# REXJJ/high-fidelity-pointcloud-fusion

Hardware: AMD Instinct MI355X
Metric: Mpts/s fused into 1 mm voxel grid (higher is better)
Workload: dtype f64

## Files before the change

### high-fidelity-pointcloud-fusion_amd/csrc/hfpf.hip

```cpp
#include <hip/hip_runtime.h>

#include <cstring>

#include <rocprim/rocprim.hpp>

#include <dlfcn.h>
#include <sched.h>
#include <sys/mman.h>

#if !defined(__HIP_DEVICE_COMPILE__)
#include <emmintrin.h>
#endif
#include <algorithm>
#include <atomic>
#include <condition_variable>
#include <cmath>
#include <cstdarg>
#include <cstdio>
#include <cstdlib>
#include <cstring>
#include <mutex>
#include <string>
#include <thread>
#include <vector>
// ... 151 lines not shown
{
    return DepthLayout{d.color_bpp ? (const uint8_t*)dev_color : nullptr, color_stride, d.width, d.depth_step, d.color_step, d.depth_f32,
                       d.color_bpp, d.color_bgr, d.cx, d.cy, d.sx, d.sy, d.unit};
}

struct Knobs {
    int copy_streams = 2;
    bool update_cells = true;
    int host_batch = 4;
    int upd_shape_forced = -1;
    bool trace_shape = false;
    bool bin_spare = true;
    bool stream_replay = true;
    float bin_slack = 2.0f;
    bool clean_small_nowait = true;
    float test_bin_scale = 1.f;
    bool test_table_skip = false;
    bool mailbox = true;
    int test_dev_tile = kDevTileDefault;
    int stage_threads = 0;
};

struct Session {
    bool dirty = false;
    uint64_t n_linked[kLogRegions] = {0};
    uint64_t gate_done = 0;
    bool pend_valid = false;
    uint64_t direct_linked = 0;
    bool normals_possible = false;
    uint32_t next_frame_id = 0;
    bool poisoned = false;
    std::string poison_msg;
    bool bin_have_hist = false;
    bool bin_from_probe = false;
    double bin_prev_points = 0;
    uint64_t n_bricks_known = 0;
    uint64_t n_bricks_before = 0;
    unsigned long long upd_miss_seen = 0, upd_member_seen = 0;
    unsigned long long pub_seq = 0;
    uint32_t pend_n = 0, pend_first = 0;
    uint32_t pend_pts = 0;
    uint32_t pend_lay[5] = {0, 0, 0, 0, 0};
    bool pend_depth = false;
    DepthSpec pend_ds{};
    double pend_pose[kFrameSlots * 12] = {0};
    uint64_t occ_exported = 0;
    uint64_t frames_exported = 0, frames_seen = 0;
};

constexpr int kTimeIntegrate = 0, kTimeClean = 1, kTimeDetail = 2, kTimeRaycast = 5, kTimeComponents = 6, kTimeCompare = 7, kTimedIds = 8;
struct TimedId {
    std::vector<std::pair<hipEvent_t, hipEvent_t>> pending;
    double ms = 0;
    uint64_t n = 0;
// ... 20 lines not shown
    uint32_t launch_seq = 0;
    bool upd_wide = false;
    bool epoch_used = false;
    unsigned long long mbox_seq = 0;
    int stage_next = 0, fslot_next = 0;

    Tables t;
    hipStream_t stream = nullptr;
    hipStream_t copy_stream = nullptr;
    hipStream_t copy_more[3] = {nullptr, nullptr, nullptr};
    std::vector<void*> allocs;
    uint64_t device_bytes = 0;
    unsigned long long* h_ctr = nullptr;
    unsigned long long* h_log_ctr = nullptr;
    unsigned long long* mbox = nullptr;
    std::vector<DevBuf*> bufs;
    DevBuf pend_a{bufs}, pend_b{bufs};
    StageSlot stage[kStageSlots];
    FrameSlot fslot[kFrameSlots];
    void* ring_d = nullptr;
    size_t ring_cap = 0;
    hipEvent_t busy_ev = nullptr;
    bool busy_pending = false;
    void* xfer_pin[2] = {nullptr, nullptr};
    hipEvent_t xfer_ev[2] = {nullptr, nullptr};
    StagePool* stage_pool = nullptr;
    DevBuf sort_tmp{bufs}, keys_a{bufs}, keys_b{bufs}, vals_a{bufs}, vals_b{bufs}, rows_dev{bufs};
    DevBuf probe_a{bufs}, probe_b{bufs}, probe_c{bufs}, probe_d{bufs}, probe_e{bufs}, probe_f{bufs};
    DevBuf result_out{bufs};
    DevBuf zbuf{bufs}, render_pose{bufs}, render_out{bufs};
// ... 104 lines not shown
    return HFPF_OK;
}

inline unsigned blocks_for(uint64_t n, unsigned bs) { return (unsigned)std::max<uint64_t>(1, (n + bs - 1) / bs); }

__global__ void k_set_ctr(unsigned long long* ctr, int idx, unsigned long long v) { ctr[idx] = v; }
__global__ void k_set_ctr3(unsigned long long* ctr, int i0, unsigned long long v0, int i1, unsigned long long v1, int i2, unsigned long long v2)
{
    ctr[i0] = v0;
    ctr[i1] = v1;
    if (i2 >= 0) ctr[i2] = v2;
}

constexpr int kMboxLogWords = 5;
constexpr int kMboxWords = C_COUNT + kLogRegions * kMboxLogWords;
__global__ __launch_bounds__(256) void k_publish_counters(const unsigned long long* __restrict__ ctr, const unsigned long long* __restrict__ log_ctr,
                                                          unsigned long long* mbox, unsigned long long seq)
{
    const unsigned i = threadIdx.x;
    if (i < (unsigned)C_COUNT) mbox[i] = ctr[i];
    for (unsigned w = i; w < (unsigned)(kLogRegions * kMboxLogWords); w += blockDim.x) mbox[C_COUNT + w] = log_ctr[(w / kMboxLogWords) * 16 + (w % kMboxLogWords)];
    __threadfence_system();
    __syncthreads();
    if (i == 0) __hip_atomic_store(&mbox[kMboxWords + 7], seq, __ATOMIC_RELEASE, __HIP_MEMORY_SCOPE_SYSTEM);
}

int read_counters(hfpf_handle* h)
{
    if (h->mbox) {
        unsigned long long seq = h->ss.pub_seq;
        h->ss.pub_seq = 0;
        if (seq == 0) {
            seq = ++h->mbox_seq;
            k_publish_counters<<<1, 256, 0, h->stream>>>(h->t.ctr, h->t.log_ctr, h->mbox, seq);
            HIPCHK(h, hipGetLastError());
        }
        volatile unsigned long long* flag = h->mbox + kMboxWords + 7;
        for (uint64_t spins = 1;; spins++) {
            if (__atomic_load_n(flag, __ATOMIC_ACQUIRE) == seq) break;
            __builtin_ia32_pause();
            if ((spins & 0xFFFF) == 0) {
                const hipError_t q = hipStreamQuery(h->stream);
                if (q != hipSuccess && q != hipErrorNotReady) HIPCHK(h, q);
                if (q == hipSuccess && __atomic_load_n(flag, __ATOMIC_ACQUIRE) != seq)
                    return fail(h, HFPF_ERR_HIP, "counter mailbox: the stream drained without publishing sequence %llu", seq);
            }
        }
        memcpy(h->h_ctr, h->mbox, C_COUNT * sizeof(unsigned long long));
        for (int r = 0; r < kLogRegions; r++)
            for (int w = 0; w < kMboxLogWords; w++) h->h_log_ctr[r * 16 + w] = h->mbox[C_COUNT + r * kMboxLogWords + w];
    } else {
        HIPCHK(h, hipMemcpyAsync(h->h_ctr, h->t.ctr, C_COUNT * sizeof(unsigned long long), hipMemcpyDeviceToHost, h->stream));
        HIPCHK(h, hipMemcpyAsync(h->h_log_ctr, h->t.log_ctr, kLogRegions * 16 * sizeof(unsigned long long), hipMemcpyDeviceToHost, h->stream));
        HIPCHK(h, hipStreamSynchronize(h->stream));
    }
    unsigned long long total = 0;
    for (int r = 0; r < kLogRegions; r++) total += std::min<unsigned long long>(h->h_log_ctr[r * 16], h->t.log_region_cap);
    h->h_ctr[C_LOG] = total;
    unsigned long long replayed = 0;
    for (int r = 0; r < kLogRegions; r++) replayed += h->h_log_ctr[r * 16 + 1];
    h->h_ctr[C_REPLAY_MEMBER] = replayed;
    unsigned long long upd_tested = 0, upd_member = 0;
    for (int r = 0; r < kLogRegions; r++) {
        upd_tested += h->h_log_ctr[r * 16 + 2];
        upd_member += h->h_log_ctr[r * 16 + 3];
// ... 33 lines not shown
float stat_scale_for(double bound) { return (float)std::ldexp(1.0, 26 - (int)std::floor(std::log2(bound))); }

Knobs read_knobs()
{
    Knobs k;
    if (const char* cs = getenv("HFPF_COPY_STREAMS")) k.copy_streams = std::max(1, std::min(atoi(cs), 4));
    const char* uf = getenv("HFPF_UPDATE_FORM");
    k.update_cells = !(uf && uf[0] == 'p');
    if (const char* hb = getenv("HFPF_HOST_BATCH")) k.host_batch = std::max(1, std::min(atoi(hb), kFrameSlots));
    if (const char* us = getenv("HFPF_UPD_SHAPE")) k.upd_shape_forced = std::max(0, std::min(atoi(us), 1));
    if (const char* tr = getenv("HFPF_TRACE_SHAPE")) k.trace_shape = tr[0] != '0';
    if (const char* sp = getenv("HFPF_BIN_SPARE")) k.bin_spare = sp[0] != '0';
    if (const char* sr = getenv("HFPF_STREAM_REPLAY")) k.stream_replay = sr[0] != '0';
    if (const char* bs = getenv("HFPF_BIN_SLACK")) k.bin_slack = std::max(1.0f, std::min(4.0f, (float)atof(bs)));
    if (const char* nw = getenv("HFPF_CLEAN_NOWAIT")) k.clean_small_nowait = nw[0] != '0';
    if (const char* bs = getenv("HFPF_TEST_BIN_SCALE")) k.test_bin_scale = std::max(0.f, std::min(1.f, (float)atof(bs)));
    const char* ts = getenv("HFPF_TEST_TABLE_SKIP");
    k.test_table_skip = ts && ts[0] == '1';
    if (const char* dt = getenv("HFPF_TEST_DEV_TILE")) k.test_dev_tile = std::max(8, std::min(atoi(dt), kDevTileMax));
    const char* mb = getenv("HFPF_MAILBOX");
    k.mailbox = !mb || mb[0] != '0';
    int cores = (int)std::thread::hardware_concurrency();
    cpu_set_t set;
    if (sched_getaffinity(0, sizeof set, &set) == 0) cores = std::min(cores > 0 ? cores : 1 << 20, CPU_COUNT(&set));
    const char* st = getenv("HFPF_STAGE_THREADS");
    k.stage_threads = st ? std::max(0, std::min(atoi(st), 15)) : std::max(0, std::min(7, cores / 2 - 1));
    return k;
}

int setup_params(hfpf_handle* h)
// ... 70 lines not shown
        memcpy(&g.d2_max, &lo_b, 4);
    }
    const double dir_entries = (double)g.bdim[0] * (double)g.bdim[1] * (double)g.bdim[2];
    if (dir_entries > 4.0e9) return fail(h, HFPF_ERR_BAD_CONFIG, "brick directory too large (%.3g entries)", dir_entries);
    h->dir_entries = (size_t)dir_entries;
    return HFPF_OK;
}

int reset_state(hfpf_handle* h, uint64_t bricks_used = ~0ull, uint64_t normals_used = ~0ull)
{
    Tables& t = h->t;
    hipStream_t s = h->stream;
    const uint64_t nb = std::min<uint64_t>(bricks_used, t.max_bricks);
    const uint64_t nsl = std::min<uint64_t>(h->n_slots, (nb + 1) * (uint64_t)kBrickCells);
    const uint64_t nn = std::min<uint64_t>(normals_used, t.max_normals);
    HIPCHK(h, hipMemsetAsync(t.dir, 0, h->dir_entries * 4, s));
    HIPCHK(h, hipMemsetAsync(t.info, 0, nsl * 8, s));
    HIPCHK(h, hipMemsetAsync(t.first_frame, 0xFF, nsl * 4, s));
    HIPCHK(h, hipMemsetAsync(t.buf_head, 0, nsl * 4 * kChains, s));
    HIPCHK(h, hipMemsetAsync(t.stat_id, 0, nsl * 4, s));
    HIPCHK(h, hipMemsetAsync(t.pre_dep, 0, nsl * 4, s));
    HIPCHK(h, hipMemsetAsync(t.dep_tmp, 0, nsl * 4, s));
    HIPCHK(h, hipMemsetAsync(t.occ_mask, 0, (nb + 1) * 8 * 8, s));
    HIPCHK(h, hipMemsetAsync(t.stats, 0, (nn + 1) * kStatWords * 8, s));
    HIPCHK(h, hipMemsetAsync(t.nd_mask, 0, (nb + 1) * 8 * 2 * 8, s));
    HIPCHK(h, hipMemsetAsync(t.ctr, 0, C_COUNT * 8, s));
    HIPCHK(h, hipMemsetAsync(t.log_ctr, 0, kLogRegions * 16 * 8, s));
    HIPCHK(h, hipMemsetAsync(t.bin_fill, 0, 2 * (t.max_bricks + 2) * 4, s));
    HIPCHK(h, hipMemsetAsync(t.bin_off, 0, 2 * (t.max_bricks + 2) * 4, s));
    HIPCHK(h, hipMemsetAsync(t.bin_capb, 0, 2 * (t.max_bricks + 2) * 4, s));
// ... 79 lines not shown
#define HFPF_SORT_BLOCK_ITEMS 4
#endif
using sort_config = rocprim::radix_sort_config<rocprim::default_config, rocprim::merge_sort_config<512, 1024, HFPF_SORT_BLOCK_ITEMS>, rocprim::default_config>;

template <typename Fn>
int with_sort_tmp(hfpf_handle* h, Fn&& fn)
{
    size_t bytes = 0;
    HIPCHK(h, fn((void*)nullptr, bytes));
    if (int rc = scratch(h, h->sort_tmp, bytes)) return rc;
    bytes = h->sort_tmp.bytes;
    HIPCHK(h, fn(h->sort_tmp.p, bytes));
    return HFPF_OK;
}

int sort_keys_u64(hfpf_handle* h, uint64_t* in, uint64_t* out, uint64_t n, unsigned bits = 0)
{
    const unsigned kb = bits ? bits : h->g.key_bits;
    return with_sort_tmp(h, [&](void* tmp, size_t& bytes) { return rocprim::radix_sort_keys<sort_config>(tmp, bytes, in, out, (size_t)n, 0, kb, h->stream); });
}

int sort_keys_u32(hfpf_handle* h, uint32_t* in, uint32_t* out, uint64_t n, unsigned bits = 32)
{
    return with_sort_tmp(h, [&](void* tmp, size_t& bytes) { return rocprim::radix_sort_keys<sort_config>(tmp, bytes, in, out, (size_t)n, 0, bits, h->stream); });
}

int sort_pairs_u64(hfpf_handle* h, uint64_t* kin, uint64_t* kout, uint32_t* vin, uint32_t* vout, uint64_t n, unsigned bits = 0)
{
    const unsigned kb = bits ? bits : h->g.key_bits;
    return with_sort_tmp(h, [&](void* tmp, size_t& bytes) {
        return rocprim::radix_sort_pairs<sort_config>(tmp, bytes, kin, kout, vin, vout, (size_t)n, 0, kb, h->stream);
    });
}

// ... 35 lines not shown
    if (s.cap < n_frames) {
        if (s.h_pose) {
            HIPCHK(h, hipHostFree(s.h_pose));
            HIPCHK(h, hipFree(s.d_pose));
            s.h_pose = nullptr, s.d_pose = nullptr, s.cap = 0;
        }
        const uint32_t cap = std::max<uint32_t>(n_frames, 64);
        const size_t bytes = (size_t)cap * (12 * sizeof(double) + sizeof(uint32_t));
        HIPCHK(h, hipHostMalloc((void**)&s.h_pose, bytes, hipHostMallocDefault));
        HIPCHK(h, hipMalloc((void**)&s.d_pose, bytes));
        s.cap = cap;
    }
    s.h_ids = reinterpret_cast<uint32_t*>(s.h_pose + 12 * (size_t)n_frames);
    s.d_ids = reinterpret_cast<uint32_t*>(s.d_pose + 12 * (size_t)n_frames);
    *out = &s;
    return HFPF_OK;
}

int pick_update_shape(hfpf_handle* h, double points, uint32_t nb)
{
    (void)points;
    (void)nb;
    if (h->knobs.upd_shape_forced >= 0) return h->knobs.upd_shape_forced;
    const unsigned long long miss = h->h_ctr[C_TABLE_MISS], member = h->h_ctr[C_DEP_MEMBER] + h->h_ctr[C_REPLAY_MEMBER];
    if (h->knobs.trace_shape)
        fprintf(stderr, "hfpf: update shape window: %llu table misses, %llu members (%llu of them replayed so far), %s\n", miss - std::min(miss, h->ss.upd_miss_seen),
                member - std::min(member, h->ss.upd_member_seen), h->h_ctr[C_REPLAY_MEMBER], h->upd_wide ? "wide" : "dense");
    if (!h->upd_wide && miss > h->ss.upd_miss_seen && (miss - h->ss.upd_miss_seen) * 500ull > member - std::min(member, h->ss.upd_member_seen)) h->upd_wide = true;
    h->ss.upd_miss_seen = miss;
    h->ss.upd_member_seen = member;
// ... 113 lines not shown
    return timed.file(id);
}

int integrate_device_locked(hfpf_handle* h, const void* dev_base, uint32_t n_frames, uint64_t frame_stride, uint32_t n_points,
                            uint32_t point_step, uint32_t off_x, uint32_t off_y, uint32_t off_z, uint32_t off_rgb, const double* poses,
                            const uint32_t* frame_ids, const DepthLayout* dl = nullptr)
{
    if (!dev_base || !poses || n_frames == 0) return fail(h, HFPF_ERR_BAD_ARG, "integrate: null buffer/poses or zero frames");
    if (n_points == 0) return HFPF_OK;
    const FrameLayout lay{point_step, off_x, off_y, off_z, off_rgb};
    if (!dl && (((uintptr_t)dev_base & 3) || (frame_stride & 3))) return fail(h, HFPF_ERR_BAD_ARG, "integrate: fields must be 4-byte aligned");
    int rc;
    if (!dl && (rc = check_cloud_layout(h, "integrate", lay, true))) return rc;
    if (n_frames > 65535) return fail(h, HFPF_ERR_BAD_ARG, "integrate: at most 65535 frames per call");
    h->ss.pub_seq = 0;
    StageSlot* s = nullptr;
    if ((rc = acquire_stage(h, n_frames, &s))) return rc;
    memcpy(s->h_pose, poses, (size_t)n_frames * 12 * sizeof(double));
    for (uint32_t f = 0; f < n_frames; f++) {
        const uint32_t id = frame_ids ? frame_ids[f] : h->ss.next_frame_id + f;
        if (id >= h->t.max_frames) return fail(h, HFPF_ERR_CAPACITY, "frame id %u >= max_frames %llu", id, (unsigned long long)h->t.max_frames);
        s->h_ids[f] = id;
    }
    if (!frame_ids) h->ss.next_frame_id += n_frames;
    HIPCHK(h, hipMemcpyAsync(s->d_pose, s->h_pose, (size_t)n_frames * (12 * sizeof(double) + sizeof(uint32_t)), hipMemcpyHostToDevice, h->stream));

    const int form = dl ? kFormDepth : packed16(lay, dev_base, true, frame_stride) ? kFormPacked16 : kFormStrided;
    const dim3 block(256);
    const uint64_t n_tiles = (uint64_t)blocks_for(n_points, 256) * n_frames;
    const uint32_t fw = dl ? dl->width : h->cfg.frame_width;
// ... 80 lines not shown
    const uint32_t log_rot = (uint32_t)((h->launch_seq++ * 17u) & (kLogRegions - 1));
    struct DetailGuard {
        hfpf_handle* h;
        size_t first;
        bool done = false;
        ~DetailGuard()
        {
            if (done) return;
            while (h->ev_detail.size() > first) {
                h->ev_free.push_back(h->ev_detail.back());
                h->ev_detail.pop_back();
            }
        }
    } detail_guard{h, h->ev_detail.size()};
    uint8_t detail_ran = 1;
    auto detail_mark = [&]() -> hipError_t {
        if (!h->timing_detail) return hipSuccess;
        hipEvent_t e = nullptr;
        if (hipError_t r = pooled_event(h, &e)) return r;
        h->ev_detail.push_back(e);
        return hipEventRecord(e, h->stream);
    };
    HIPCHK(h, detail_mark());
    launch_integrate(grid, bin, n_frames, log_rot, 0);
    if (!bin) {
        for (int k = 0; k < 3; k++) HIPCHK(h, detail_mark());
    } else {
        {
            const unsigned ogrid = (unsigned)std::min<uint64_t>(blocks_for((uint64_t)n_points * n_frames, 256), 8ull * 256);
            with_color(color, [&](auto C) { hipLaunchKernelGGL(k_integrate_overflow<C>, dim3(ogrid), dim3(256), 0, h->stream, h->g, h->t, log_rot); });
        }
        HIPCHK(h, detail_mark());
        if (have_plan) {
            if (h->h_ctr[C_NORMALS] > 0 || h->ss.normals_possible) {
                detail_ran |= 2;
                if (h->knobs.update_cells) {
                    const int shape = pick_update_shape(h, (double)n_points * n_frames, nb);
                    launch_update_cells<false>(color, shape == 1, h->stream, h->g, h->t, nb);
                } else {
                    with_color(color, [&](auto C) { hipLaunchKernelGGL(k_update<C>, dim3(nb), dim3(kUpdThreads), 0, h->stream, h->g, h->t, nb); });
                }
            }
            HIPCHK(h, detail_mark());
            detail_ran |= 4;
            with_color(color, [&](auto C) { hipLaunchKernelGGL(k_buffer<C>, dim3(nb), dim3(256), 0, h->stream, h->g, h->t, nb); });
            HIPCHK(h, detail_mark());
        } else {
            HIPCHK(h, detail_mark());
            HIPCHK(h, detail_mark());
        }
        h->ss.bin_have_hist = true;
        h->ss.bin_prev_points = (double)n_points * n_frames;
    }
    HIPCHK(h, hipGetLastError());
    if (h->timing_detail) h->ev_detail_ran.push_back(detail_ran);
    detail_guard.done = true;
    if ((rc = timed.file(kTimeIntegrate))) return rc;
    HIPCHK(h, hipEventRecord(s->done, h->stream));
    s->pending = true;
    h->ss.dirty = true;
    h->frames_integrated += n_frames;
    if (h->mbox && n_frames >= 4) {
        h->ss.pub_seq = ++h->mbox_seq;
        k_publish_counters<<<1, 256, 0, h->stream>>>(h->t.ctr, h->t.log_ctr, h->mbox, h->ss.pub_seq);
        HIPCHK(h, hipGetLastError());
    } else {
        h->ss.pub_seq = 0;
    }
    return HFPF_OK;
}

int resolve_timing(hfpf_handle* h)
{
    bool pending = !h->ev_detail.empty();
    for (const TimedId& t : h->timed) pending = pending || !t.pending.empty();
    if (!pending) return HFPF_OK;
    HIPCHK(h, hipStreamSynchronize(h->stream));
    for (TimedId& t : h->timed) {
        for (auto& pr : t.pending) {
            float ms = 0.f;
            HIPCHK(h, hipEventElapsedTime(&ms, pr.first, pr.second));
            t.ms += (double)ms;
            t.n++;
            h->ev_free.push_back(pr.first);
            h->ev_free.push_back(pr.second);
        }
        t.pending.clear();
    }
    for (size_t c = 0; 4 * c + 3 < h->ev_detail.size() && c < h->ev_detail_ran.size(); c++) {
        for (int k = 0; k < 3; k++) {
            if (!(h->ev_detail_ran[c] & (1u << k))) continue;
            float ms = 0.f;
            HIPCHK(h, hipEventElapsedTime(&ms, h->ev_detail[4 * c + k], h->ev_detail[4 * c + k + 1]));
            h->timed[kTimeDetail + k].ms += (double)ms;
            h->timed[kTimeDetail + k].n++;
        }
    }
    for (hipEvent_t e : h->ev_detail) h->ev_free.push_back(e);
    h->ev_detail.clear();
    h->ev_detail_ran.clear();
    return HFPF_OK;
}


typedef struct ncclComm* ncclComm_t_;
typedef struct { char internal[128]; } ncclUniqueId_;
enum { ncclSuccess_ = 0 };
enum { ncclChar_ = 0, ncclUint64_ = 5 };
// ... 149 lines not shown
    uint64_t maxc = 0;
    for (int r = 0; r < h->world; r++) maxc = std::max<uint64_t>(maxc, h->h_counts[r]);
    if (maxc == 0) return HFPF_OK;
    if (maxc > h->ex_cap_records) {
        const uint64_t new_cap = maxc + maxc / 4;
        const int grc = grow_exchange_buffers_locked(h, new_cap, n_mine);
        std::vector<unsigned long long> counts(h->h_counts, h->h_counts + h->world);
        if ((rc = dist_status_gather_locked(h, grc, new_cap, "growth of the exchange buffers", nullptr))) return rc;
        std::copy(counts.begin(), counts.end(), h->h_counts);
        h->ex_cap_records = new_cap;
    }
    NCCLCHK(h, g_rccl.AllGather(h->ex_send.p, h->ex_recv.p, maxc * sizeof(EpochRec), ncclChar_, (ncclComm_t_)h->comm, h->stream));
    return import_gathered_locked(h, h->ex_recv.p, maxc * sizeof(EpochRec), h->world, h->rank, h->h_counts);
}

void launch_gate(hfpf_handle* h, const uint32_t* cells_a, uint64_t n_a, const uint32_t* cells_b, uint64_t n_b, uint32_t* pend_out)
{
    const uint64_t n = n_a + n_b;
    if (n >= (1ull << 20))
        hipLaunchKernelGGL(k_gate<4>, dim3(blocks_for(n, 256 * 4)), dim3(256), 0, h->stream, h->g, h->t, cells_a, n_a, cells_b, n_b, pend_out);
    else
        hipLaunchKernelGGL(k_gate<1>, dim3(blocks_for(n, 256)), dim3(256), 0, h->stream, h->g, h->t, cells_a, n_a, cells_b, n_b, pend_out);
}

int clean_locked(hfpf_handle* h, int pre_rc)
{
    Tables& t = h->t;
    hipStream_t s = h->stream;
    int rc;
    if (h->dist_on && (rc = dist_exchange_locked(h, pre_rc))) return rc;
    if (pre_rc) return pre_rc;
    if ((rc = read_counters(h))) return rc;
    if ((rc = check_device_errors(h))) return rc;
    const uint64_t n_occ = std::min<uint64_t>(h->h_ctr[C_OCC], t.max_occ);
    const uint64_t n_normals = h->h_ctr[C_NORMALS];
    const uint64_t n_pend = h->ss.pend_valid ? h->h_ctr[C_PEND] : 0;
    h->ss.occ_exported = n_occ;
    h->ss.frames_exported = std::max(h->ss.frames_exported, h->ss.frames_seen);
    h->ss.dirty = false;
    h->clean_passes++;

    {
        LinkRanges lr;
        uint64_t max_new = 0;
        for (int r = 0; r < kLogRegions; r++) {
            const uint64_t n_r = std::min<uint64_t>(h->h_log_ctr[r * 16], t.log_region_cap);
            const uint64_t base = (uint64_t)r * t.log_region_cap;
// ... 6 lines not shown
            hipLaunchKernelGGL(k_link_log, dim3(blocks_for(max_new, 256), kLogRegions), dim3(256), 0, s, t, lr);
            HIPCHK(h, hipGetLastError());
        }
        h->ss.direct_linked = h->h_ctr[C_BUFFERED];
    }
    if (n_occ == 0) return HFPF_OK;

    const uint64_t n_new_occ = n_occ - std::min(n_occ, h->ss.gate_done);
    const uint64_t n_in = n_pend + n_new_occ;
    if (n_in == 0) return HFPF_OK;
    if ((rc = scratch(h, h->pend_b, n_in * 4))) return rc;
    if ((rc = scratch(h, h->keys_a, n_in * 8))) return rc;
    const uint64_t reg_ub = (2ull * (uint64_t)h->g.K + 1ull) * n_in;
    const uint64_t live_ub = std::min<uint64_t>(h->h_ctr[C_REG], t.max_reg) + std::min<uint64_t>(h->h_ctr[C_PREREG], t.max_reg);
    bool full = h->h_ctr[C_DEP] + 2 * live_ub + 2 * reg_ub + n_new_occ > t.max_dep;
    hipLaunchKernelGGL(k_clean_begin, dim3(blocks_for(n_in, 256)), dim3(256), 0, s, t, n_in, (const uint32_t*)(t.occ_list + h->ss.gate_done), n_new_occ, full ? 1u : 0u);
    launch_gate(h, (const uint32_t*)h->pend_a.p, n_pend, (const uint32_t*)(t.occ_list + h->ss.gate_done), n_new_occ, (uint32_t*)h->pend_b.p);
    HIPCHK(h, hipGetLastError());
    h->ss.gate_done = n_occ;
    h->ss.normals_possible = true;
    swap(h->pend_a, h->pend_b);
    h->ss.pend_valid = true;

    const unsigned cand_bits = HFPF_MORTON_IDS ? 3u * std::max(h->g.key_sy, std::max(h->g.key_sx - h->g.key_sy, h->g.key_bits - h->g.key_sx)) : h->g.key_bits;
    if ((rc = sort_keys_u64(h, t.cand_key, (uint64_t*)h->keys_a.p, n_in, cand_bits))) return rc;
    hipLaunchKernelGGL(k_normal, dim3(blocks_for(n_in, 128)), dim3(128), 0, s, h->g, t, (const uint64_t*)h->keys_a.p, kCountOnDevice, n_normals);
    const bool reg_small = n_in < (1ull << 18);
    const uint64_t reg_tile = 256ull * (reg_small ? kRegTilesSmall : kRegTilesLarge);
    const uint64_t reg_blocks = ((n_in + reg_tile - 1) / reg_tile) * (2ull * (uint64_t)h->g.K + 1ull);
    const uint32_t count_deps = full ? 0u : 1u;
    if (reg_small) hipLaunchKernelGGL(k_register<kRegTilesSmall>, dim3((unsigned)std::max<uint64_t>(reg_blocks, 1)), dim3(256), 0, s, h->g, t, kCountOnDevice, n_normals, count_deps);
    else hipLaunchKernelGGL(k_register<kRegTilesLarge>, dim3((unsigned)std::max<uint64_t>(reg_blocks, 1)), dim3(256), 0, s, h->g, t, kCountOnDevice, n_normals, count_deps);
    HIPCHK(h, hipGetLastError());
    uint64_t n_reg = 0, n_pre = 0, inc_touched = 0;
    const uint64_t reg_first = std::min<uint64_t>(h->h_ctr[C_REG], t.max_reg);
    const bool no_wait = !full && reg_ub < (1ull << 21) && h->knobs.clean_small_nowait;
    if (!full) {
        hipLaunchKernelGGL(k_depinc_offsets, dim3(blocks_for(reg_ub, 256 * kListTiles)), dim3(256), 0, s, t, kCountOnDevice);
        hipLaunchKernelGGL(k_depinc_fill, dim3(blocks_for(reg_ub, 256)), dim3(256), 0, s, t, reg_first, kCountOnDevice);
        HIPCHK(h, hipGetLastError());
        if (no_wait) {
            with_color(t.color, [&](auto C) {
                hipLaunchKernelGGL(k_replay<C>, dim3(blocks_for(reg_ub * kChains, 256)), dim3(256), 0, s, h->g, t, (const uint32_t*)t.touched_list, 1u, 0u,
                                   kCountOnDevice, n_normals);
            });
            HIPCHK(h, hipGetLastError());
            return HFPF_OK;
        }
// ... 96 lines not shown
    *out = nullptr;
    hfpf_handle* h = new hfpf_handle();
    h->cfg = *cfg;
    h->knobs = read_knobs();
    auto bail = [&](int rc) {
        g_create_error = h->err;
        for (void* p : h->allocs) (void)hipFree(p);
        for (DevBuf* b : h->bufs)
            if (b->p) (void)hipFree(b->p);
        if (h->h_ctr) (void)hipHostFree(h->h_ctr);
        if (h->h_log_ctr) (void)hipHostFree(h->h_log_ctr);
        if (h->mbox) (void)hipHostFree(h->mbox);
        if (h->copy_stream) (void)hipStreamDestroy(h->copy_stream);
        for (hipStream_t cs : h->copy_more)
            if (cs) (void)hipStreamDestroy(cs);
        if (h->stream) (void)hipStreamDestroy(h->stream);
        delete h;
        return rc;
    };
    int rc = setup_params(h);
    if (rc) return bail(rc);
    int ndev = 0;
    hipError_t e = hipGetDeviceCount(&ndev);
    if (e != hipSuccess || ndev <= 0) return bail(fail(h, HFPF_ERR_HIP, "no HIP device available (%s); this engine has no CPU path", hipGetErrorString(e)));
    if (cfg->device < 0 || cfg->device >= ndev) return bail(fail(h, HFPF_ERR_BAD_CONFIG, "device %d out of range (%d devices)", cfg->device, ndev));
    if ((e = hipSetDevice(cfg->device)) != hipSuccess) return bail(fail(h, HFPF_ERR_HIP, "hipSetDevice: %s", hipGetErrorString(e)));
    if ((e = hipStreamCreateWithFlags(&h->stream, hipStreamNonBlocking)) != hipSuccess) return bail(fail(h, HFPF_ERR_HIP, "hipStreamCreate: %s", hipGetErrorString(e)));
    if ((e = hipStreamCreateWithFlags(&h->copy_stream, hipStreamNonBlocking)) != hipSuccess) return bail(fail(h, HFPF_ERR_HIP, "hipStreamCreate: %s", hipGetErrorString(e)));
    for (int k = 0; k + 1 < h->knobs.copy_streams; k++)
        if ((e = hipStreamCreateWithFlags(&h->copy_more[k], hipStreamNonBlocking)) != hipSuccess) return bail(fail(h, HFPF_ERR_HIP, "hipStreamCreate: %s", hipGetErrorString(e)));
    if ((e = hipHostMalloc((void**)&h->h_ctr, C_COUNT * sizeof(unsigned long long), hipHostMallocDefault)) != hipSuccess)
        return bail(fail(h, HFPF_ERR_HIP, "hipHostMalloc: %s", hipGetErrorString(e)));
    memset(h->h_ctr, 0, C_COUNT * sizeof(unsigned long long));
    if ((e = hipHostMalloc((void**)&h->h_log_ctr, kLogRegions * 16 * sizeof(unsigned long long), hipHostMallocDefault)) != hipSuccess)
        return bail(fail(h, HFPF_ERR_HIP, "hipHostMalloc: %s", hipGetErrorString(e)));
    memset(h->h_log_ctr, 0, kLogRegions * 16 * sizeof(unsigned long long));
    if (h->knobs.mailbox) {
        if ((e = hipHostMalloc((void**)&h->mbox, (kMboxWords + 8) * sizeof(unsigned long long), hipHostMallocCoherent | hipHostMallocMapped)) != hipSuccess)
            return bail(fail(h, HFPF_ERR_HIP, "hipHostMalloc (mailbox): %s", hipGetErrorString(e)));
        memset(h->mbox, 0, (kMboxWords + 8) * sizeof(unsigned long long));
    }
    {
        int per_cu = 0, cus = 0;
        hipDeviceProp_t prop;
        if (hipGetDeviceProperties(&prop, cfg->device) == hipSuccess) cus = prop.multiProcessorCount;
        if (hipOccupancyMaxActiveBlocksPerMultiprocessor(&per_cu, h->binned ? k_integrate<true, false, true> : k_integrate<true, false, false>, 256, 0) != hipSuccess) per_cu = 4;
        h->integrate_grid = std::max(1, per_cu) * std::max(1, cus);
    }
    if ((rc = alloc_tables(h))) return bail(rc);
    {
        const uint64_t n0 = h->cfg.max_normals;
        if ((rc = scratch(h, h->keys_a, n0 * 8)) || (rc = scratch(h, h->keys_b, n0 * 8)) || (rc = scratch(h, h->vals_a, n0 * 4)) ||
            (rc = scratch(h, h->vals_b, n0 * 4)) || (rc = scratch(h, h->pend_b, n0 * 4)) || (rc = scratch(h, h->sort_tmp, n0 * 16)))
            return bail(rc);
        if (h->cfg.max_call_points && h->binned) {
// ... 11 lines not shown
            if (h->xfer_pin[0]) (void)hipHostFree(h->xfer_pin[0]);
            h->xfer_pin[0] = nullptr;
            break;
        }
    }
    if ((e = hipStreamSynchronize(h->stream)) != hipSuccess) return bail(fail(h, HFPF_ERR_HIP, "sync after init: %s", hipGetErrorString(e)));
    *out = h;
    return HFPF_OK;
}

int hfpf_destroy(hfpf_handle* h)
{
    if (!h) return HFPF_OK;
    (void)hipSetDevice(h->cfg.device);
    (void)hipStreamSynchronize(h->stream);
    for (void* p : h->allocs) (void)hipFree(p);
    for (DevBuf* b : h->bufs)
        if (b->p) (void)hipFree(b->p);
    if (h->comm && g_rccl.CommDestroy) (void)g_rccl.CommDestroy((ncclComm_t_)h->comm);
    if (h->h_counts) (void)hipHostFree(h->h_counts);
    for (auto& s : h->stage) {
        if (s.h_pose) (void)hipHostFree(s.h_pose);
        if (s.d_pose) (void)hipFree(s.d_pose);
        if (s.done) (void)hipEventDestroy(s.done);
    }
    delete h->stage_pool;
    h->stage_pool = nullptr;
    for (int k = 0; k < 2; k++) {
        if (h->xfer_pin[k]) (void)hipHostFree(h->xfer_pin[k]);
        if (h->xfer_ev[k]) (void)hipEventDestroy(h->xfer_ev[k]);
// ... 12 lines not shown
    for (hipStream_t cs : h->copy_more)
        if (cs) {
            (void)hipStreamSynchronize(cs);
            (void)hipStreamDestroy(cs);
        }
    for (TimedId& t : h->timed)
        for (auto& pr : t.pending) {
            (void)hipEventDestroy(pr.first);
            (void)hipEventDestroy(pr.second);
        }
    for (auto e : h->ev_detail) (void)hipEventDestroy(e);
    for (auto e : h->ev_free) (void)hipEventDestroy(e);
    if (h->h_ctr) (void)hipHostFree(h->h_ctr);
    if (h->h_log_ctr) (void)hipHostFree(h->h_log_ctr);
    if (h->mbox) (void)hipHostFree(h->mbox);
    if (h->stream) (void)hipStreamDestroy(h->stream);
    delete h;
    return HFPF_OK;
}

int hfpf_get_dims(const hfpf_handle* h, int32_t dims[3], double* resolution)
{
    if (!h) return HFPF_ERR_BAD_ARG;
    if (dims) memcpy(dims, h->g.dim, 3 * sizeof(int32_t));
    if (resolution) *resolution = h->g.res;
    return HFPF_OK;
}

static int flush_pending_locked(hfpf_handle* h);

// ... 3176 lines not shown
```

### high-fidelity-pointcloud-fusion_amd/csrc/kernels.hpp

```cpp
#pragma once
#include <type_traits>

#include "stats.hpp"

namespace hfpf {

typedef float vf4 __attribute__((ext_vector_type(4)));

struct FrameLayout {
    uint32_t point_step, off_x, off_y, off_z, off_rgb;
};

struct DepthLayout {
    const uint8_t* color;
    uint64_t color_stride;
    uint32_t width, depth_step, color_step;
    uint32_t depth_f32;
    uint32_t color_bpp;
    uint32_t color_bgr;
    float cx, cy, sx, sy, unit;
};

template <bool WANT_RGB>
__device__ __forceinline__ vf4 depth_fetch(const uint8_t* __restrict__ dimg, const uint8_t* __restrict__ cimg, const DepthLayout& L, uint32_t i)
// ... 1236 lines not shown
    block_reserve_tiles<TILES>(&t.ctr[C_CAND], n_pass, ci, trs);
    block_reserve_tiles<TILES>(&t.ctr[C_PEND], n_pend, pi, trs);
#pragma unroll
    for (int tt = 0; tt < TILES; tt++) {
        if (n_pass[tt]) t.cand_key[ci[tt]] = key_[tt];
        if (n_pend[tt]) pend_out[pi[tt]] = slot_[tt];
    }
}

__device__ __forceinline__ uint64_t cand_count(const Tables& t, uint64_t base)
{
    const uint64_t n = t.ctr[C_CAND];
    const uint64_t room = t.max_normals > base ? t.max_normals - base : 0;
    return n < room ? n : room;
}
__global__ __launch_bounds__(256) void k_clean_begin(const Tables t, const uint64_t n_in, const uint32_t* __restrict__ new_cells, const uint64_t n_new,
                                                     const uint32_t lists_only)
{
    const uint64_t i = (uint64_t)blockIdx.x * blockDim.x + threadIdx.x;
    if (i < n_in) t.cand_key[i] = ~0ull;
    if (i == 0) {
        t.ctr[C_CAND] = 0;
        t.ctr[C_PEND] = 0;
        t.ctr[C_TOUCHED] = 0;
    }
    if (i < (uint64_t)kLogRegions) t.log_ctr[i * 16 + 4] = 0;
    if ((uint64_t)blockIdx.x * blockDim.x >= n_new) return;
    uint32_t slot = 0, nid = 0;
    if (i < n_new) {
        slot = new_cells[i];
        nid = t.pre_dep[slot];
    }
    __shared__ BlockReserveScratch brs;
    const unsigned long long li = block_reserve(&t.ctr[C_PREREG], nid != 0, brs);
    const unsigned long long off = lists_only ? 0ull : block_reserve(&t.ctr[C_DEP], nid != 0, brs);
    if (!nid) return;
    if (li < t.max_reg) t.prereg_list[li] = slot;
    else atomicOr(&t.ctr[C_ERR], (unsigned long long)E_REG);
    set_dep_flag(t, slot);
    if (lists_only) return;
    if (off >= t.max_dep) {
        atomicOr(&t.ctr[C_ERR], (unsigned long long)E_DEP);
        return;
    }
    t.dep[off] = make_dep_entry(t, nid);
    t.info[slot] = (t.info[slot] & 3ull) | (1ull << kDepCntShift) | ((uint64_t)off << kDepOffShift);
}

__global__ __launch_bounds__(128) void k_normal(const GridParams g, const Tables t, const uint64_t* __restrict__ sorted_keys,
                                                const uint64_t n_cand_arg, const uint64_t base)
{
    const uint64_t n_cand = n_cand_arg == kCountOnDevice ? cand_count(t, base) : n_cand_arg;
    const uint64_t r = (uint64_t)blockIdx.x * blockDim.x + threadIdx.x;
    if (r == 0 && n_cand_arg == kCountOnDevice) {
        if (t.ctr[C_CAND] > n_cand) atomicOr(&t.ctr[C_ERR], (unsigned long long)E_NORMALS);
        t.ctr[C_NORMALS] = base + n_cand;
    }
    if (r >= n_cand) return;
    int32_t x, y, z;
    uint64_t key = sorted_keys[r];
    if (HFPF_MORTON_IDS) {
// ... 2584 lines not shown
```

Baseline: 28120.

## Overlap clean front half with update-cells kernel on a second stream

Result: faster. 29420 (median of 6 runs) (+4.6%).

```diff
diff --git a/high-fidelity-pointcloud-fusion_amd/csrc/hfpf.hip b/high-fidelity-pointcloud-fusion_amd/csrc/hfpf.hip
--- a/high-fidelity-pointcloud-fusion_amd/csrc/hfpf.hip
+++ b/high-fidelity-pointcloud-fusion_amd/csrc/hfpf.hip
@@ -189,6 +189,8 @@
     bool stream_replay = true;
     float bin_slack = 2.0f;
     bool clean_small_nowait = true;
+    bool clean_overlap = true;
+    bool trace_clean = false;
     float test_bin_scale = 1.f;
     bool test_table_skip = false;
     bool mailbox = true;
@@ -213,6 +215,8 @@
     uint64_t n_bricks_before = 0;
     unsigned long long upd_miss_seen = 0, upd_member_seen = 0;
     unsigned long long pub_seq = 0;
+    unsigned long long early_seq = 0;
+    unsigned long long win_seq = 0;
     uint32_t pend_n = 0, pend_first = 0;
     uint32_t pend_pts = 0;
     uint32_t pend_lay[5] = {0, 0, 0, 0, 0};
@@ -263,6 +267,8 @@
     unsigned long long* h_ctr = nullptr;
     unsigned long long* h_log_ctr = nullptr;
     unsigned long long* mbox = nullptr;
+    hipStream_t front_stream = nullptr;
+    hipEvent_t ev_ready = nullptr, ev_front = nullptr;
     std::vector<DevBuf*> bufs;
     DevBuf pend_a{bufs}, pend_b{bufs};
     StageSlot stage[kStageSlots];
@@ -397,6 +403,7 @@
 
 constexpr int kMboxLogWords = 5;
 constexpr int kMboxWords = C_COUNT + kLogRegions * kMboxLogWords;
+constexpr int kMboxSlotWords = (kMboxWords + 8 + 7) & ~7;
 __global__ __launch_bounds__(256) void k_publish_counters(const unsigned long long* __restrict__ ctr, const unsigned long long* __restrict__ log_ctr,
                                                           unsigned long long* mbox, unsigned long long seq)
 {
@@ -408,30 +415,39 @@
     if (i == 0) __hip_atomic_store(&mbox[kMboxWords + 7], seq, __ATOMIC_RELEASE, __HIP_MEMORY_SCOPE_SYSTEM);
 }
 
-int read_counters(hfpf_handle* h)
+int await_mailbox(hfpf_handle* h, const unsigned long long* box, unsigned long long seq)
+{
+    const unsigned long long* flag = box + kMboxWords + 7;
+    for (uint64_t spins = 1;; spins++) {
+        if (__atomic_load_n(flag, __ATOMIC_ACQUIRE) == seq) break;
+        __builtin_ia32_pause();
+        if ((spins & 0xFFFF) == 0) {
+            const hipError_t q = hipStreamQuery(h->stream);
+            if (q != hipSuccess && q != hipErrorNotReady) HIPCHK(h, q);
+            if (q == hipSuccess && __atomic_load_n(flag, __ATOMIC_ACQUIRE) != seq)
+                return fail(h, HFPF_ERR_HIP, "counter mailbox: the stream drained without publishing sequence %llu", seq);
+        }
+    }
+    return HFPF_OK;
+}
+
+int read_counters(hfpf_handle* h, bool early = false)
 {
     if (h->mbox) {
-        unsigned long long seq = h->ss.pub_seq;
+        unsigned long long seq = early ? h->ss.early_seq : h->ss.pub_seq;
+        const unsigned long long* box = h->mbox + (early ? kMboxSlotWords : 0);
+        h->ss.win_seq = early ? h->ss.pub_seq : 0;
         h->ss.pub_seq = 0;
+        h->ss.early_seq = 0;
         if (seq == 0) {
             seq = ++h->mbox_seq;
             k_publish_counters<<<1, 256, 0, h->stream>>>(h->t.ctr, h->t.log_ctr, h->mbox, seq);
             HIPCHK(h, hipGetLastError());
         }
-        volatile unsigned long long* flag = h->mbox + kMboxWords + 7;
-        for (uint64_t spins = 1;; spins++) {
-            if (__atomic_load_n(flag, __ATOMIC_ACQUIRE) == seq) break;
-            __builtin_ia32_pause();
-            if ((spins & 0xFFFF) == 0) {
-                const hipError_t q = hipStreamQuery(h->stream);
-                if (q != hipSuccess && q != hipErrorNotReady) HIPCHK(h, q);
-                if (q == hipSuccess && __atomic_load_n(flag, __ATOMIC_ACQUIRE) != seq)
-                    return fail(h, HFPF_ERR_HIP, "counter mailbox: the stream drained without publishing sequence %llu", seq);
-            }
-        }
-        memcpy(h->h_ctr, h->mbox, C_COUNT * sizeof(unsigned long long));
+        if (int rc = await_mailbox(h, box, seq)) return rc;
+        memcpy(h->h_ctr, box, C_COUNT * sizeof(unsigned long long));
         for (int r = 0; r < kLogRegions; r++)
-            for (int w = 0; w < kMboxLogWords; w++) h->h_log_ctr[r * 16 + w] = h->mbox[C_COUNT + r * kMboxLogWords + w];
+            for (int w = 0; w < kMboxLogWords; w++) h->h_log_ctr[r * 16 + w] = box[C_COUNT + r * kMboxLogWords + w];
     } else {
         HIPCHK(h, hipMemcpyAsync(h->h_ctr, h->t.ctr, C_COUNT * sizeof(unsigned long long), hipMemcpyDeviceToHost, h->stream));
         HIPCHK(h, hipMemcpyAsync(h->h_log_ctr, h->t.log_ctr, kLogRegions * 16 * sizeof(unsigned long long), hipMemcpyDeviceToHost, h->stream));
@@ -495,6 +511,8 @@
     if (const char* sr = getenv("HFPF_STREAM_REPLAY")) k.stream_replay = sr[0] != '0';
     if (const char* bs = getenv("HFPF_BIN_SLACK")) k.bin_slack = std::max(1.0f, std::min(4.0f, (float)atof(bs)));
     if (const char* nw = getenv("HFPF_CLEAN_NOWAIT")) k.clean_small_nowait = nw[0] != '0';
+    if (const char* co = getenv("HFPF_CLEAN_OVERLAP")) k.clean_overlap = co[0] != '0';
+    if (const char* tc = getenv("HFPF_TRACE_CLEAN")) k.trace_clean = tc[0] != '0';
     if (const char* bs = getenv("HFPF_TEST_BIN_SCALE")) k.test_bin_scale = std::max(0.f, std::min(1.f, (float)atof(bs)));
     const char* ts = getenv("HFPF_TEST_TABLE_SKIP");
     k.test_table_skip = ts && ts[0] == '1';
@@ -595,6 +613,7 @@
     const uint64_t nb = std::min<uint64_t>(bricks_used, t.max_bricks);
     const uint64_t nsl = std::min<uint64_t>(h->n_slots, (nb + 1) * (uint64_t)kBrickCells);
     const uint64_t nn = std::min<uint64_t>(normals_used, t.max_normals);
+    if (h->front_stream) HIPCHK(h, hipStreamSynchronize(h->front_stream));
     HIPCHK(h, hipMemsetAsync(t.dir, 0, h->dir_entries * 4, s));
     HIPCHK(h, hipMemsetAsync(t.info, 0, nsl * 8, s));
     HIPCHK(h, hipMemsetAsync(t.first_frame, 0xFF, nsl * 4, s));
@@ -704,10 +723,11 @@
     return HFPF_OK;
 }
 
-int sort_keys_u64(hfpf_handle* h, uint64_t* in, uint64_t* out, uint64_t n, unsigned bits = 0)
+int sort_keys_u64(hfpf_handle* h, uint64_t* in, uint64_t* out, uint64_t n, unsigned bits = 0, hipStream_t on = nullptr)
 {
     const unsigned kb = bits ? bits : h->g.key_bits;
-    return with_sort_tmp(h, [&](void* tmp, size_t& bytes) { return rocprim::radix_sort_keys<sort_config>(tmp, bytes, in, out, (size_t)n, 0, kb, h->stream); });
+    const hipStream_t st = on ? on : h->stream;
+    return with_sort_tmp(h, [&](void* tmp, size_t& bytes) { return rocprim::radix_sort_keys<sort_config>(tmp, bytes, in, out, (size_t)n, 0, kb, st); });
 }
 
 int sort_keys_u32(hfpf_handle* h, uint32_t* in, uint32_t* out, uint64_t n, unsigned bits = 32)
@@ -773,6 +793,24 @@
     s.h_ids = reinterpret_cast<uint32_t*>(s.h_pose + 12 * (size_t)n_frames);
     s.d_ids = reinterpret_cast<uint32_t*>(s.d_pose + 12 * (size_t)n_frames);
     *out = &s;
+    return HFPF_OK;
+}
+
+int window_from_final(hfpf_handle* h)
+{
+    const unsigned long long seq = h->ss.win_seq;
+    h->ss.win_seq = 0;
+    if (!seq || !h->mbox) return HFPF_OK;
+    if (int rc = await_mailbox(h, h->mbox, seq)) return rc;
+    unsigned long long member = h->mbox[C_DEP_MEMBER], tested = h->mbox[C_DEP_TESTED];
+    for (int r = 0; r < kLogRegions; r++) {
+        tested += h->mbox[C_COUNT + r * kMboxLogWords + 2];
+        member += h->mbox[C_COUNT + r * kMboxLogWords + 3];
+    }
+    h->h_ctr[C_DEP_TESTED] = tested;
+    h->h_ctr[C_DEP_MEMBER] = member;
+    h->h_ctr[C_TABLE_MISS] = h->mbox[C_TABLE_MISS];
+    h->h_ctr[C_UPD_ROUNDS] = h->mbox[C_UPD_ROUNDS];
     return HFPF_OK;
 }
 
@@ -916,6 +954,7 @@
     if (!dl && (rc = check_cloud_layout(h, "integrate", lay, true))) return rc;
     if (n_frames > 65535) return fail(h, HFPF_ERR_BAD_ARG, "integrate: at most 65535 frames per call");
     h->ss.pub_seq = 0;
+    h->ss.early_seq = 0;
     StageSlot* s = nullptr;
     if ((rc = acquire_stage(h, n_frames, &s))) return rc;
     memcpy(s->h_pose, poses, (size_t)n_frames * 12 * sizeof(double));
@@ -1026,6 +1065,7 @@
         }
     } detail_guard{h, h->ev_detail.size()};
     uint8_t detail_ran = 1;
+    unsigned long long early_seq = 0;
     auto detail_mark = [&]() -> hipError_t {
         if (!h->timing_detail) return hipSuccess;
         hipEvent_t e = nullptr;
@@ -1044,9 +1084,25 @@
         }
         HIPCHK(h, detail_mark());
         if (have_plan) {
-            if (h->h_ctr[C_NORMALS] > 0 || h->ss.normals_possible) {
+            const bool update = h->h_ctr[C_NORMALS] > 0 || h->ss.normals_possible;
+            const bool buffer_first = update && h->knobs.clean_overlap && h->mbox && n_frames >= 4 && !h->dist_on;
+            auto launch_buffer = [&]() {
+                detail_ran |= 4;
+                with_color(color, [&](auto C) { hipLaunchKernelGGL(k_buffer<C>, dim3(nb), dim3(256), 0, h->stream, h->g, h->t, nb); });
+            };
+            if (buffer_first) {
+                detail_ran |= 8;
+                launch_buffer();
+                early_seq = ++h->mbox_seq;
+                k_publish_counters<<<1, 256, 0, h->stream>>>(h->t.ctr, h->t.log_ctr, h->mbox + kMboxSlotWords, early_seq);
+                HIPCHK(h, hipGetLastError());
+                HIPCHK(h, hipEventRecord(h->ev_ready, h->stream));
+                HIPCHK(h, detail_mark());
+            }
+            if (update) {
                 detail_ran |= 2;
                 if (h->knobs.update_cells) {
+                    if ((rc = window_from_final(h))) return rc;
                     const int shape = pick_update_shape(h, (double)n_points * n_frames, nb);
                     launch_update_cells<false>(color, shape == 1, h->stream, h->g, h->t, nb);
                 } else {
@@ -1054,9 +1110,10 @@
                 }
             }
             HIPCHK(h, detail_mark());
-            detail_ran |= 4;
-            with_color(color, [&](auto C) { hipLaunchKernelGGL(k_buffer<C>, dim3(nb), dim3(256), 0, h->stream, h->g, h->t, nb); });
-            HIPCHK(h, detail_mark());
+            if (!buffer_first) {
+                launch_buffer();
+                HIPCHK(h, detail_mark());
+            }
         } else {
             HIPCHK(h, detail_mark());
             HIPCHK(h, detail_mark());
@@ -1073,9 +1130,11 @@
     h->ss.dirty = true;
     h->frames_integrated += n_frames;
     if (h->mbox && n_frames >= 4) {
+        if ((rc = window_from_final(h))) return rc;
         h->ss.pub_seq = ++h->mbox_seq;
         k_publish_counters<<<1, 256, 0, h->stream>>>(h->t.ctr, h->t.log_ctr, h->mbox, h->ss.pub_seq);
         HIPCHK(h, hipGetLastError());
+        h->ss.early_seq = early_seq;
     } else {
         h->ss.pub_seq = 0;
     }
@@ -1102,8 +1161,9 @@
     for (size_t c = 0; 4 * c + 3 < h->ev_detail.size() && c < h->ev_detail_ran.size(); c++) {
         for (int k = 0; k < 3; k++) {
             if (!(h->ev_detail_ran[c] & (1u << k))) continue;
+            const int at = (k && (h->ev_detail_ran[c] & 8u)) ? 3 - k : k;
             float ms = 0.f;
-            HIPCHK(h, hipEventElapsedTime(&ms, h->ev_detail[4 * c + k], h->ev_detail[4 * c + k + 1]));
+            HIPCHK(h, hipEventElapsedTime(&ms, h->ev_detail[4 * c + at], h->ev_detail[4 * c + at + 1]));
             h->timed[kTimeDetail + k].ms += (double)ms;
             h->timed[kTimeDetail + k].n++;
         }
@@ -1283,13 +1343,13 @@
     return import_gathered_locked(h, h->ex_recv.p, maxc * sizeof(EpochRec), h->world, h->rank, h->h_counts);
 }
 
-void launch_gate(hfpf_handle* h, const uint32_t* cells_a, uint64_t n_a, const uint32_t* cells_b, uint64_t n_b, uint32_t* pend_out)
+void launch_gate(hfpf_handle* h, hipStream_t s, const uint32_t* cells_a, uint64_t n_a, const uint32_t* cells_b, uint64_t n_b, uint32_t* pend_out)
 {
     const uint64_t n = n_a + n_b;
     if (n >= (1ull << 20))
-        hipLaunchKernelGGL(k_gate<4>, dim3(blocks_for(n, 256 * 4)), dim3(256), 0, h->stream, h->g, h->t, cells_a, n_a, cells_b, n_b, pend_out);
+        hipLaunchKernelGGL(k_gate<4>, dim3(blocks_for(n, 256 * 4)), dim3(256), 0, s, h->g, h->t, cells_a, n_a, cells_b, n_b, pend_out);
     else
-        hipLaunchKernelGGL(k_gate<1>, dim3(blocks_for(n, 256)), dim3(256), 0, h->stream, h->g, h->t, cells_a, n_a, cells_b, n_b, pend_out);
+        hipLaunchKernelGGL(k_gate<1>, dim3(blocks_for(n, 256)), dim3(256), 0, s, h->g, h->t, cells_a, n_a, cells_b, n_b, pend_out);
 }
 
 int clean_locked(hfpf_handle* h, int pre_rc)
@@ -1299,7 +1359,8 @@
     int rc;
     if (h->dist_on && (rc = dist_exchange_locked(h, pre_rc))) return rc;
     if (pre_rc) return pre_rc;
-    if ((rc = read_counters(h))) return rc;
+    const bool early = h->knobs.clean_overlap && !h->dist_on && h->binned && h->mbox && h->ss.pub_seq && h->ss.early_seq;
+    if ((rc = read_counters(h, early))) return rc;
     if ((rc = check_device_errors(h))) return rc;
     const uint64_t n_occ = std::min<uint64_t>(h->h_ctr[C_OCC], t.max_occ);
     const uint64_t n_normals = h->h_ctr[C_NORMALS];
@@ -1336,8 +1397,19 @@
     const uint64_t reg_ub = (2ull * (uint64_t)h->g.K + 1ull) * n_in;
     const uint64_t live_ub = std::min<uint64_t>(h->h_ctr[C_REG], t.max_reg) + std::min<uint64_t>(h->h_ctr[C_PREREG], t.max_reg);
     bool full = h->h_ctr[C_DEP] + 2 * live_ub + 2 * reg_ub + n_new_occ > t.max_dep;
-    hipLaunchKernelGGL(k_clean_begin, dim3(blocks_for(n_in, 256)), dim3(256), 0, s, t, n_in, (const uint32_t*)(t.occ_list + h->ss.gate_done), n_new_occ, full ? 1u : 0u);
-    launch_gate(h, (const uint32_t*)h->pend_a.p, n_pend, (const uint32_t*)(t.occ_list + h->ss.gate_done), n_new_occ, (uint32_t*)h->pend_b.p);
+    const bool overlap = early && !full;
+    const uint32_t* new_cells = (const uint32_t*)(t.occ_list + h->ss.gate_done);
+    if (h->knobs.trace_clean)
+        fprintf(stderr, "hfpf: clean pass %llu: %llu candidates, front half %s\n", (unsigned long long)h->clean_passes, (unsigned long long)n_in,
+                overlap ? "beside the update kernel" : "on the engine's stream");
+    if (overlap) {
+        s = h->front_stream;
+        HIPCHK(h, hipStreamWaitEvent(s, h->ev_ready, 0));
+        hipLaunchKernelGGL(k_clean_front, dim3(blocks_for(n_in, 256)), dim3(256), 0, s, t, n_in);
+    } else {
+        hipLaunchKernelGGL(k_clean_begin, dim3(blocks_for(n_in, 256)), dim3(256), 0, s, t, n_in, new_cells, n_new_occ, full ? 1u : 0u);
+    }
+    launch_gate(h, s, (const uint32_t*)h->pend_a.p, n_pend, new_cells, n_new_occ, (uint32_t*)h->pend_b.p);
     HIPCHK(h, hipGetLastError());
     h->ss.gate_done = n_occ;
     h->ss.normals_possible = true;
@@ -1345,7 +1417,7 @@
     h->ss.pend_valid = true;
 
     const unsigned cand_bits = HFPF_MORTON_IDS ? 3u * std::max(h->g.key_sy, std::max(h->g.key_sx - h->g.key_sy, h->g.key_bits - h->g.key_sx)) : h->g.key_bits;
-    if ((rc = sort_keys_u64(h, t.cand_key, (uint64_t*)h->keys_a.p, n_in, cand_bits))) return rc;
+    if ((rc = sort_keys_u64(h, t.cand_key, (uint64_t*)h->keys_a.p, n_in, cand_bits, s))) return rc;
     hipLaunchKernelGGL(k_normal, dim3(blocks_for(n_in, 128)), dim3(128), 0, s, h->g, t, (const uint64_t*)h->keys_a.p, kCountOnDevice, n_normals);
     const bool reg_small = n_in < (1ull << 18);
     const uint64_t reg_tile = 256ull * (reg_small ? kRegTilesSmall : kRegTilesLarge);
@@ -1354,6 +1426,12 @@
     if (reg_small) hipLaunchKernelGGL(k_register<kRegTilesSmall>, dim3((unsigned)std::max<uint64_t>(reg_blocks, 1)), dim3(256), 0, s, h->g, t, kCountOnDevice, n_normals, count_deps);
     else hipLaunchKernelGGL(k_register<kRegTilesLarge>, dim3((unsigned)std::max<uint64_t>(reg_blocks, 1)), dim3(256), 0, s, h->g, t, kCountOnDevice, n_normals, count_deps);
     HIPCHK(h, hipGetLastError());
+    if (overlap) {
+        HIPCHK(h, hipEventRecord(h->ev_front, s));
+        s = h->stream;
+        HIPCHK(h, hipStreamWaitEvent(s, h->ev_front, 0));
+        if (n_new_occ) hipLaunchKernelGGL(k_clean_file, dim3(blocks_for(n_new_occ, 256)), dim3(256), 0, s, t, new_cells, n_new_occ);
+    }
     uint64_t n_reg = 0, n_pre = 0, inc_touched = 0;
     const uint64_t reg_first = std::min<uint64_t>(h->h_ctr[C_REG], t.max_reg);
     const bool no_wait = !full && reg_ub < (1ull << 21) && h->knobs.clean_small_nowait;
@@ -1480,6 +1558,9 @@
         if (h->copy_stream) (void)hipStreamDestroy(h->copy_stream);
         for (hipStream_t cs : h->copy_more)
             if (cs) (void)hipStreamDestroy(cs);
+        if (h->ev_ready) (void)hipEventDestroy(h->ev_ready);
+        if (h->ev_front) (void)hipEventDestroy(h->ev_front);
+        if (h->front_stream) (void)hipStreamDestroy(h->front_stream);
         if (h->stream) (void)hipStreamDestroy(h->stream);
         delete h;
         return rc;
@@ -1495,6 +1576,9 @@
     if ((e = hipStreamCreateWithFlags(&h->copy_stream, hipStreamNonBlocking)) != hipSuccess) return bail(fail(h, HFPF_ERR_HIP, "hipStreamCreate: %s", hipGetErrorString(e)));
     for (int k = 0; k + 1 < h->knobs.copy_streams; k++)
         if ((e = hipStreamCreateWithFlags(&h->copy_more[k], hipStreamNonBlocking)) != hipSuccess) return bail(fail(h, HFPF_ERR_HIP, "hipStreamCreate: %s", hipGetErrorString(e)));
+    if ((e = hipStreamCreateWithFlags(&h->front_stream, hipStreamNonBlocking)) != hipSuccess) return bail(fail(h, HFPF_ERR_HIP, "hipStreamCreate: %s", hipGetErrorString(e)));
+    if ((e = hipEventCreateWithFlags(&h->ev_ready, hipEventDisableTiming)) != hipSuccess || (e = hipEventCreateWithFlags(&h->ev_front, hipEventDisableTiming)) != hipSuccess)
+        return bail(fail(h, HFPF_ERR_HIP, "hipEventCreate: %s", hipGetErrorString(e)));
     if ((e = hipHostMalloc((void**)&h->h_ctr, C_COUNT * sizeof(unsigned long long), hipHostMallocDefault)) != hipSuccess)
         return bail(fail(h, HFPF_ERR_HIP, "hipHostMalloc: %s", hipGetErrorString(e)));
     memset(h->h_ctr, 0, C_COUNT * sizeof(unsigned long long));
@@ -1502,9 +1586,9 @@
         return bail(fail(h, HFPF_ERR_HIP, "hipHostMalloc: %s", hipGetErrorString(e)));
     memset(h->h_log_ctr, 0, kLogRegions * 16 * sizeof(unsigned long long));
     if (h->knobs.mailbox) {
-        if ((e = hipHostMalloc((void**)&h->mbox, (kMboxWords + 8) * sizeof(unsigned long long), hipHostMallocCoherent | hipHostMallocMapped)) != hipSuccess)
+        if ((e = hipHostMalloc((void**)&h->mbox, 2 * kMboxSlotWords * sizeof(unsigned long long), hipHostMallocCoherent | hipHostMallocMapped)) != hipSuccess)
             return bail(fail(h, HFPF_ERR_HIP, "hipHostMalloc (mailbox): %s", hipGetErrorString(e)));
-        memset(h->mbox, 0, (kMboxWords + 8) * sizeof(unsigned long long));
+        memset(h->mbox, 0, 2 * kMboxSlotWords * sizeof(unsigned long long));
     }
     {
         int per_cu = 0, cus = 0;
@@ -1546,6 +1630,7 @@
     if (!h) return HFPF_OK;
     (void)hipSetDevice(h->cfg.device);
     (void)hipStreamSynchronize(h->stream);
+    if (h->front_stream) (void)hipStreamSynchronize(h->front_stream);
     for (void* p : h->allocs) (void)hipFree(p);
     for (DevBuf* b : h->bufs)
         if (b->p) (void)hipFree(b->p);
@@ -1588,6 +1673,9 @@
     if (h->h_ctr) (void)hipHostFree(h->h_ctr);
     if (h->h_log_ctr) (void)hipHostFree(h->h_log_ctr);
     if (h->mbox) (void)hipHostFree(h->mbox);
+    if (h->ev_ready) (void)hipEventDestroy(h->ev_ready);
+    if (h->ev_front) (void)hipEventDestroy(h->ev_front);
+    if (h->front_stream) (void)hipStreamDestroy(h->front_stream);
     if (h->stream) (void)hipStreamDestroy(h->stream);
     delete h;
     return HFPF_OK;
diff --git a/high-fidelity-pointcloud-fusion_amd/csrc/kernels.hpp b/high-fidelity-pointcloud-fusion_amd/csrc/kernels.hpp
--- a/high-fidelity-pointcloud-fusion_amd/csrc/kernels.hpp
+++ b/high-fidelity-pointcloud-fusion_amd/csrc/kernels.hpp
@@ -1274,10 +1274,8 @@
     const uint64_t room = t.max_normals > base ? t.max_normals - base : 0;
     return n < room ? n : room;
 }
-__global__ __launch_bounds__(256) void k_clean_begin(const Tables t, const uint64_t n_in, const uint32_t* __restrict__ new_cells, const uint64_t n_new,
-                                                     const uint32_t lists_only)
-{
-    const uint64_t i = (uint64_t)blockIdx.x * blockDim.x + threadIdx.x;
+__device__ __forceinline__ void clean_front(const Tables& t, const uint64_t i, const uint64_t n_in)
+{
     if (i < n_in) t.cand_key[i] = ~0ull;
     if (i == 0) {
         t.ctr[C_CAND] = 0;
@@ -1285,6 +1283,9 @@
         t.ctr[C_TOUCHED] = 0;
     }
     if (i < (uint64_t)kLogRegions) t.log_ctr[i * 16 + 4] = 0;
+}
+__device__ __forceinline__ void clean_file(const Tables& t, const uint64_t i, const uint32_t* __restrict__ new_cells, const uint64_t n_new, const uint32_t lists_only)
+{
     if ((uint64_t)blockIdx.x * blockDim.x >= n_new) return;
     uint32_t slot = 0, nid = 0;
     if (i < n_new) {
@@ -1305,6 +1306,21 @@
     }
     t.dep[off] = make_dep_entry(t, nid);
     t.info[slot] = (t.info[slot] & 3ull) | (1ull << kDepCntShift) | ((uint64_t)off << kDepOffShift);
+}
+__global__ __launch_bounds__(256) void k_clean_begin(const Tables t, const uint64_t n_in, const uint32_t* __restrict__ new_cells, const uint64_t n_new,
+                                                     const uint32_t lists_only)
+{
+    const uint64_t i = (uint64_t)blockIdx.x * blockDim.x + threadIdx.x;
+    clean_front(t, i, n_in);
+    clean_file(t, i, new_cells, n_new, lists_only);
+}
+__global__ __launch_bounds__(256) void k_clean_front(const Tables t, const uint64_t n_in)
+{
+    clean_front(t, (uint64_t)blockIdx.x * blockDim.x + threadIdx.x, n_in);
+}
+__global__ __launch_bounds__(256) void k_clean_file(const Tables t, const uint32_t* __restrict__ new_cells, const uint64_t n_new)
+{
+    clean_file(t, (uint64_t)blockIdx.x * blockDim.x + threadIdx.x, new_cells, n_new, 0u);
 }
 
 __global__ __launch_bounds__(128) void k_normal(const GridParams g, const Tables t, const uint64_t* __restrict__ sorted_keys,
```
